# OliBomby/Mapperatorinator

Hardware: AMD Instinct MI355X
Metric: beatmap event-tokens/sec (mel + osuT5 encoder + greedy AR decode), whole job (higher is better)
Workload: dtype bf16; 1 GPU; osuT5-base bf16, batch=32 x 10 s chunks per GPU, 384 greedy tokens per chunk, mel+encoder+cross-KV+AR decode (BASELINE configs[1]); chunks_per_gpu=32, src_frames=1251, vocab=1849, parallelism=chunk-sharded x1, all_gather of token streams

## Files before the change

### mapperatorinator_amd/csrc/decode_kernels.hpp

```cpp
#pragma once
#include <type_traits>

#include "internal.hpp"

namespace mh {
namespace dec {

#ifdef MH_PHASE_STAMPS
__device__ unsigned long long g_stamps[16 * 16 * 2];
#define MH_STAMP0() unsigned long long mh_t0_ = 0; if (blockIdx.x == 0 && threadIdx.x == 0) mh_t0_ = clock64()
#define MH_STAMP(kid, i)                                                              \
  do {                                                                                \
    if (blockIdx.x == 0 && threadIdx.x == 0) {                                        \
      atomicAdd(&g_stamps[((kid) * 16 + (i)) * 2], (unsigned long long)clock64() - mh_t0_); \
      atomicAdd(&g_stamps[((kid) * 16 + (i)) * 2 + 1], 1ull);                         \
    }                                                                                 \
  } while (0)
#else
#define MH_STAMP0() do {} while (0)
#define MH_STAMP(kid, i) do {} while (0)
#endif
enum { KID_GEMV = 0 , KID_SELF = 10, KID_CROSS = 11, KID_SAMPLE = 12 };

typedef __attribute__((ext_vector_type(4))) unsigned int u32x4_t;
typedef __attribute__((ext_vector_type(2))) unsigned int u32x2_t;
template <typename T> __device__ inline void load8_stream(const T* p, float (&o)[8]);
template <> __device__ inline void load8_stream<bf16_t>(const bf16_t* p, float (&o)[8]) {
  const u32x4_t v = __builtin_nontemporal_load(reinterpret_cast<const u32x4_t*>(p));
#pragma unroll
  for (int i = 0; i < 4; ++i) {
    o[2 * i] = __uint_as_float(v[i] << 16);
    o[2 * i + 1] = __uint_as_float(v[i] & 0xffff0000u);
  }
}
template <> __device__ inline void load8_stream<float>(const float* p, float (&o)[8]) {
  const u32x4_t a = __builtin_nontemporal_load(reinterpret_cast<const u32x4_t*>(p));
  const u32x4_t b = __builtin_nontemporal_load(reinterpret_cast<const u32x4_t*>(p + 4));
#pragma unroll
  for (int i = 0; i < 4; ++i) { o[i] = __uint_as_float(a[i]); o[4 + i] = __uint_as_float(b[i]); }
}
struct fp8_t { uint8_t v; };
typedef __attribute__((ext_vector_type(2))) float f32x2_t;
template <> __device__ inline void load8_stream<fp8_t>(const fp8_t* p, float (&o)[8]) {
  const u32x2_t v = __builtin_nontemporal_load(reinterpret_cast<const u32x2_t*>(p));
#pragma unroll
  for (int i = 0; i < 2; ++i) {
    const f32x2_t lo = __builtin_amdgcn_cvt_pk_f32_fp8((int)v[i], false);
    const f32x2_t hi = __builtin_amdgcn_cvt_pk_f32_fp8((int)v[i], true);
    o[4 * i] = lo[0]; o[4 * i + 1] = lo[1]; o[4 * i + 2] = hi[0]; o[4 * i + 3] = hi[1];
  }
}
template <typename T> __device__ inline void store8(T* p, const float (&o)[8]);
template <> __device__ inline void store8<bf16_t>(bf16_t* p, const float (&o)[8]) {
  uint32_t w[4];
#pragma unroll
  for (int i = 0; i < 4; ++i) w[i] = pack_bf16x2(o[2 * i], o[2 * i + 1]);
  *reinterpret_cast<uint4*>(p) = make_uint4(w[0], w[1], w[2], w[3]);
}
template <> __device__ inline void store8<float>(float* p, const float (&o)[8]) {
  *reinterpret_cast<float4*>(p) = make_float4(o[0], o[1], o[2], o[3]);
  *reinterpret_cast<float4*>(p + 4) = make_float4(o[4], o[5], o[6], o[7]);
}

template <typename T> __device__ inline void store4(T* p, float a, float b, float c, float d);
template <> __device__ inline void store4<bf16_t>(bf16_t* p, float a, float b, float c, float d) {
  *reinterpret_cast<uint2*>(p) = make_uint2(pack_bf16x2(a, b), pack_bf16x2(c, d));
}
template <> __device__ inline void store4<float>(float* p, float a, float b, float c, float d) {
  *reinterpret_cast<float4*>(p) = make_float4(a, b, c, d);
}

#define MH_LOADS_ISSUED() do {} while (0)


template <typename U>
__device__ inline void store_wt(U* p, U v) { __hip_atomic_store(p, v, __ATOMIC_RELAXED, __HIP_MEMORY_SCOPE_AGENT); }
__device__ inline void store16_wt(void* p, u32x4_t v) { asm volatile("global_store_dwordx4 %0, %1, off sc1" : : "v"(p), "v"(v) : "memory"); }
__device__ inline void store8_wt(void* p, u32x2_t v) { asm volatile("global_store_dwordx2 %0, %1, off sc1" : : "v"(p), "v"(v) : "memory"); }
template <typename TO>
__device__ inline void store_piece_wt(TO* dst, const float* v, int n, int nvalid) {
  const bool whole = nvalid == n && (reinterpret_cast<uintptr_t>(dst) & (n * sizeof(TO) - 1)) == 0;
  if (whole && sizeof(TO) == 4 && n == 4) {
    store16_wt(dst, u32x4_t{__float_as_uint(v[0]), __float_as_uint(v[1]), __float_as_uint(v[2]), __float_as_uint(v[3])});
  } else if (whole && sizeof(TO) == 2 && n == 8) {
    store16_wt(dst, u32x4_t{pack_bf16x2(v[0], v[1]), pack_bf16x2(v[2], v[3]), pack_bf16x2(v[4], v[5]), pack_bf16x2(v[6], v[7])});
  } else if (whole && sizeof(TO) == 2 && n == 4) {
    store8_wt(dst, u32x2_t{pack_bf16x2(v[0], v[1]), pack_bf16x2(v[2], v[3])});
  } else {
    for (int i = 0; i < nvalid; ++i) store_wt(dst + i, Elem<TO>::from_f32(v[i]));
  }
}

template <typename T>
__device__ inline void store_head_row_wt(T* dst, float val, float* patch) {
  const int lane = threadIdx.x & 63;
  constexpr int N = 16 / (int)sizeof(T);
  patch[lane] = val;
  __builtin_amdgcn_fence(__ATOMIC_RELEASE, "wavefront");
  __builtin_amdgcn_wave_barrier();
  __builtin_amdgcn_fence(__ATOMIC_ACQUIRE, "wavefront");
  if (lane < 64 / N) {
    float v[8];
#pragma unroll
    for (int i = 0; i < 8; ++i) v[i] = i < N ? patch[lane * N + i] : 0.f;
    store_piece_wt<T>(dst + lane * N, v, N, N);
  }
}
template <typename T>
__device__ inline void store_head_row_from_lds_wt(T* dst, const float* src, int t) {
  constexpr int N = 16 / (int)sizeof(T);
  if (t >= 0 && t < 64 / N) {
    float v[8];
#pragma unroll
    for (int i = 0; i < 8; ++i) v[i] = i < N ? src[t * N + i] : 0.f;
    store_piece_wt<T>(dst + t * N, v, N, N);
  }
}

enum { PRO_PLAIN = 0, PRO_RMSNORM = 1, PRO_LAYERNORM = 2 };
enum { SK_GEGLU = 2, SK_RESID = 3, SK_LOGITS = 4, SK_GELU_ERF = 5 };

struct SkinnyP {
  const void* A; int lda;
  const float* ln_w; float eps;
  const void* W; int ldw;
  int B, N, K;
  int nv;
  void* out; int ldo;
  float* h; int ldh;
  void* kc; void* vc;
  int H, tgt_len, inner;
  const int* pos;
  const float* bias;
  const float* ln_b;
};

template <typename T> struct VecOps;
template <> struct VecOps<bf16_t> {
  struct Raw { float4 a, b; };
  __device__ static inline Raw load_raw(const float* p) {
    Raw r;
    r.a = *reinterpret_cast<const float4*>(p);
    r.b = *reinterpret_cast<const float4*>(p + 4);
    return r;
  }
  __device__ static inline float sumsq(const Raw& x) {
    return (x.a.x * x.a.x + x.a.y * x.a.y) + (x.a.z * x.a.z + x.a.w * x.a.w) + (x.b.x * x.b.x + x.b.y * x.b.y) +
           (x.b.z * x.b.z + x.b.w * x.b.w);
  }
  __device__ static inline float sum(const Raw& x) { return (x.a.x + x.a.y) + (x.a.z + x.a.w) + (x.b.x + x.b.y) + (x.b.z + x.b.w); }
  __device__ static inline Raw centred(const Raw& x, float mu) {
    Raw r;
    r.a = make_float4(x.a.x - mu, x.a.y - mu, x.a.z - mu, x.a.w - mu);
    r.b = make_float4(x.b.x - mu, x.b.y - mu, x.b.z - mu, x.b.w - mu);
    return r;
  }
  __device__ static inline uint4 ln_frag(const Raw& x, const Raw& g, const Raw& b, float rs) {
    const uint32_t o0 = pack_bf16x2(x.a.x * rs * g.a.x + b.a.x, x.a.y * rs * g.a.y + b.a.y);
    const uint32_t o1 = pack_bf16x2(x.a.z * rs * g.a.z + b.a.z, x.a.w * rs * g.a.w + b.a.w);
    const uint32_t o2 = pack_bf16x2(x.b.x * rs * g.b.x + b.b.x, x.b.y * rs * g.b.y + b.b.y);
    const uint32_t o3 = pack_bf16x2(x.b.z * rs * g.b.z + b.b.z, x.b.w * rs * g.b.w + b.b.w);
    return make_uint4(o0, o1, o2, o3);
  }
  __device__ static inline uint4 norm_frag(const Raw& x, const Raw& g, float rs) {
    const uint32_t o0 = pack_bf16x2(g.a.x * (x.a.x * rs), g.a.y * (x.a.y * rs));
    const uint32_t o1 = pack_bf16x2(g.a.z * (x.a.z * rs), g.a.w * (x.a.w * rs));
    const uint32_t o2 = pack_bf16x2(g.b.x * (x.b.x * rs), g.b.y * (x.b.y * rs));
    const uint32_t o3 = pack_bf16x2(g.b.z * (x.b.z * rs), g.b.w * (x.b.w * rs));
    return make_uint4(o0, o1, o2, o3);
  }
  __device__ static inline f32x4_t mma(const uint4& a, const uint4& b, f32x4_t c) {
    union U { uint4 u; bf16x8_t f; };
    U ua, ub;
    ua.u = a; ub.u = b;
    return __builtin_amdgcn_mfma_f32_16x16x32_bf16(ua.f, ub.f, c, 0, 0, 0);
  }
};
template <> struct VecOps<float> {
  struct Raw { float4 a; };
  __device__ static inline Raw load_raw(const float* p) {
    Raw r;
    r.a = *reinterpret_cast<const float4*>(p);
    return r;
  }
  __device__ static inline float sumsq(const Raw& x) { return (x.a.x * x.a.x + x.a.y * x.a.y) + (x.a.z * x.a.z + x.a.w * x.a.w); }
  __device__ static inline float sum(const Raw& x) { return (x.a.x + x.a.y) + (x.a.z + x.a.w); }
  __device__ static inline Raw centred(const Raw& x, float mu) {
    Raw r;
    r.a = make_float4(x.a.x - mu, x.a.y - mu, x.a.z - mu, x.a.w - mu);
    return r;
  }
  __device__ static inline uint4 ln_frag(const Raw& x, const Raw& g, const Raw& b, float rs) {
    return make_uint4(__float_as_uint(x.a.x * rs * g.a.x + b.a.x), __float_as_uint(x.a.y * rs * g.a.y + b.a.y),
                      __float_as_uint(x.a.z * rs * g.a.z + b.a.z), __float_as_uint(x.a.w * rs * g.a.w + b.a.w));
  }
  __device__ static inline uint4 norm_frag(const Raw& x, const Raw& g, float rs) {
    return make_uint4(__float_as_uint(g.a.x * (x.a.x * rs)), __float_as_uint(g.a.y * (x.a.y * rs)),
                      __float_as_uint(g.a.z * (x.a.z * rs)), __float_as_uint(g.a.w * (x.a.w * rs)));
  }
  __device__ static inline f32x4_t mma(const uint4& a, const uint4& b, f32x4_t c) {
    c = __builtin_amdgcn_mfma_f32_16x16x4f32(__uint_as_float(a.x), __uint_as_float(b.x), c, 0, 0, 0);
    c = __builtin_amdgcn_mfma_f32_16x16x4f32(__uint_as_float(a.y), __uint_as_float(b.y), c, 0, 0, 0);
    c = __builtin_amdgcn_mfma_f32_16x16x4f32(__uint_as_float(a.z), __uint_as_float(b.z), c, 0, 0, 0);
    c = __builtin_amdgcn_mfma_f32_16x16x4f32(__uint_as_float(a.w), __uint_as_float(b.w), c, 0, 0, 0);
    return c;
  }
};

constexpr int kGemvCH = 8;

#ifndef MH_GEMV_PROBE
#define MH_GEMV_PROBE 0
#endif

#define MH_GEMV_LEAD_PARAMS const void *A_, const void *W_, float *h_, const float *lnw_, int K_, int B_, int N_, int nv_
#define MH_GEMV_LEAD_ARGS(p) (p).A, (p).W, (p).h, (p).ln_w, (p).K, (p).B, (p).N, (p).nv
template <typename T, int MF, int NWV, int PRO, int EPI, bool BIAS = false>
__global__ __launch_bounds__(NWV * 64) __attribute__((amdgpu_waves_per_eu(NWV / 4, 4)))
void gemv_kernel(MH_GEMV_LEAD_PARAMS, SkinnyP p) {
  p.A = A_; p.W = W_; p.h = h_; p.ln_w = lnw_; p.K = K_; p.lda = K_; p.ldw = K_; p.B = B_; p.N = N_; p.nv = nv_;
  if (EPI == SK_RESID) p.ldh = N_;
  constexpr int VEC = Elem<T>::kVec;
  constexpr int KB = 4 * VEC;
  constexpr int CH = kGemvCH;
  typedef typename VecOps<T>::Raw Raw;
  constexpr bool LINES = (MF == 1 && PRO == PRO_PLAIN);
  constexpr int CP = CH / 2;
  constexpr int PATCH = 16 * 144;
  constexpr bool NORM = PRO != PRO_PLAIN, LN = PRO == PRO_LAYERNORM;
  constexpr bool RLINES = (MF == 1 && NORM && sizeof(T) == 2);
  __shared__ __attribute__((aligned(16))) unsigned char Lw[(LINES || RLINES) ? NWV * PATCH : 16];
  __shared__ f32x4_t red[NWV * MF * 64];
  __shared__ float ssw[NORM ? NWV : 1][MF * 16];
  __shared__ float ssw2[LN ? NWV : 1][MF * 16];
  __shared__ __attribute__((aligned(16))) float lnw[NORM ? 1024 : 4];
  __shared__ __attribute__((aligned(16))) float lnb[LN ? 1024 : 4];

  MH_STAMP0();
  constexpr int KID = KID_GEMV + EPI * 2 + (NWV == 8 ? 1 : 0);
  const int tid = threadIdx.x, lane = tid & 63, wid = tid >> 6;
  const int l15 = lane & 15, lg = lane >> 4;
  const int nv = p.nv;
  float4 lnraw = make_float4(0.f, 0.f, 0.f, 0.f), lnbraw = make_float4(0.f, 0.f, 0.f, 0.f);
  if (NORM) {
    const int i4 = tid * 4 < p.K ? tid * 4 : 0;
    lnraw = *reinterpret_cast<const float4*>(p.ln_w + i4);
    if (LN) lnbraw = *reinterpret_cast<const float4*>(p.ln_b + i4);
  }
  int wrow, ocol;
  bool wload;
  if (EPI == SK_GEGLU) {
    ocol = blockIdx.x * 8 + (l15 & 7);
    const int oc = ocol < p.N / 2 ? ocol : p.N / 2 - 1;
    wrow = (oc >> 4) * 32 + (l15 >> 3) * 16 + (oc & 15);
    wload = true;
  } else {
    ocol = blockIdx.x * nv + l15;
    wrow = ocol < p.N ? ocol : p.N - 1;
    wload = l15 < nv;
  }
  const T* Wp = reinterpret_cast<const T*>(p.W) + (long)wrow * p.ldw + lg * VEC;
  int arow[MF];
#pragma unroll
  for (int f = 0; f < MF; ++f) arow[f] = (f * 16 + l15) < p.B ? (f * 16 + l15) : p.B - 1;

  constexpr int UPW = (MF * 4 + NWV - 1) / NWV;
  const bool col_ok = (EPI == SK_GEGLU) ? (l15 < 8 && ocol < p.N / 2) : (l15 < nv && ocol < p.N);
  float oldh[UPW];
#pragma unroll
  for (int u = 0; u < UPW; ++u) oldh[u] = 0.f;
  constexpr int PROBE = MH_GEMV_PROBE;
  float bias_v = 0.f;
  if (BIAS) bias_v = p.bias[ocol < p.N ? ocol : p.N - 1];
#define MH_LOAD_OLDH()                                                                                                        \
  do {                                                                                                                        \
    _Pragma("unroll") for (int u = 0; u < UPW; ++u) {                                                                         \
      const int unit = wid + u * NWV;                                                                                         \
      const int row = (unit >> 2) * 16 + lg * 4 + (unit & 3);                                                                 \
      if (unit < MF * 4) oldh[u] = p.h[(long)(row < p.B ? row : p.B - 1) * p.ldh + (ocol < p.N ? ocol : p.N - 1)];          \
    }                                                                                                                         \
  } while (0)
  if (EPI == SK_RESID && l15 < nv && !(PROBE & 4)) MH_LOAD_OLDH();
  f32x4_t acc[MF];
#pragma unroll
  for (int f = 0; f < MF; ++f) acc[f] = f32x4_t{0.f, 0.f, 0.f, 0.f};
  const int nkb = p.K / KB;

  auto kblock = [](int kb0, int c) -> int { return PRO == PRO_PLAIN ? 2 * (kb0 + NWV * (c >> 1)) + (c & 1) : kb0 + NWV * c; };
  int kb0 = wid;
  if constexpr (LINES) {
    const int npair = nkb >> 1;
    unsigned char* patch = Lw + wid * PATCH;
    const int r8 = lane >> 3, c16 = (lane & 7) * 16;
    const unsigned char* Ab = reinterpret_cast<const unsigned char*>(p.A) + c16;
    const long rx = (long)(r8 < p.B ? r8 : p.B - 1) * p.lda * (long)sizeof(T);
    const long ry = (long)(8 + r8 < p.B ? 8 + r8 : p.B - 1) * p.lda * (long)sizeof(T);
    for (int pw0 = wid; pw0 < npair + wid; pw0 += NWV * CP) {
      uint4 wv[CH], xa[CP], ya[CP];
#pragma unroll
      for (int c = 0; c < CH; ++c) wv[c] = make_uint4(0, 0, 0, 0);
      if (wload && !(PROBE & 2)) {
#pragma unroll
        for (int c = 0; c < CH; ++c) {
          const int pw = pw0 + NWV * (c >> 1);
          wv[c] = *reinterpret_cast<const uint4*>(Wp + (2 * (pw < npair ? pw : npair - 1) + (c & 1)) * KB);
        }
      }
#pragma unroll
      for (int cp = 0; cp < CP; ++cp) {
        const int pw = pw0 + NWV * cp;
        const long off = (long)(pw < npair ? pw : npair - 1) * 128;
        xa[cp] = *reinterpret_cast<const uint4*>(Ab + rx + off);
        ya[cp] = *reinterpret_cast<const uint4*>(Ab + ry + off);
      }
      MH_LOADS_ISSUED();
      MH_LOADS_ISSUED();
    MH_STAMP(KID, 0);
#pragma unroll
      for (int cp = 0; cp < CP; ++cp) {
        const uint32_t keep = (pw0 + NWV * cp < npair) ? 0xffffffffu : 0u;
        *reinterpret_cast<uint4*>(patch + r8 * 144 + c16) = xa[cp];
        *reinterpret_cast<uint4*>(patch + (8 + r8) * 144 + c16) = ya[cp];
#pragma unroll
        for (int j = 0; j < 2; ++j) {
          uint4 a = *reinterpret_cast<const uint4*>(patch + l15 * 144 + (j * 4 + lg) * 16);
          a = make_uint4(a.x & keep, a.y & keep, a.z & keep, a.w & keep);
          acc[0] = VecOps<T>::mma(a, wv[cp * 2 + j], acc[0]);
        }
      }
    }
  } else
  do {
    uint4 wv[CH];
    uint4 av[PRO == PRO_PLAIN ? CH : 1][PRO == PRO_PLAIN ? MF : 1];
    Raw hraw[NORM ? CH : 1][NORM ? MF : 1];
#pragma unroll
    for (int c = 0; c < CH; ++c) wv[c] = make_uint4(0, 0, 0, 0);
    if (wload && !(PROBE & 2)) {
#pragma unroll
      for (int c = 0; c < CH; ++c) {
        const int kb = kblock(kb0, c);
        wv[c] = *reinterpret_cast<const uint4*>(Wp + (kb < nkb ? kb : nkb - 1) * KB);
      }
    }
#pragma unroll
    for (int c = 0; c < CH; ++c) {
      const int kb = kblock(kb0, c);
      const int kel = (kb < nkb ? kb : nkb - 1) * KB;
      if (PROBE & 1) {
#pragma unroll
        for (int f = 0; f < MF; ++f) {
          if (PRO == PRO_PLAIN) av[c][f] = make_uint4(kel, lane, c, f);
          else hraw[c][f] = VecOps<T>::load_raw(lnw + ((kel + lane) & 1020));
        }
      } else if (PRO == PRO_PLAIN && (PROBE & 128)) {
#pragma unroll
        for (int f = 0; f < MF; ++f)
          av[c][f] = *reinterpret_cast<const uint4*>(reinterpret_cast<const T*>(p.A) + ((long)((c * NWV + wid) % (p.K * 16 / (64 * VEC))) * 64 + lane) * VEC);
      } else if (PRO == PRO_PLAIN) {
#pragma unroll
        for (int f = 0; f < MF; ++f)
          av[c][f] = *reinterpret_cast<const uint4*>(reinterpret_cast<const T*>(p.A) + (long)arow[f] * p.lda + kel + lg * VEC);
      } else if (!RLINES) {
#pragma unroll
        for (int f = 0; f < MF; ++f)
          hraw[c][f] = VecOps<T>::load_raw(reinterpret_cast<const float*>(p.A) + (long)arow[f] * p.lda + kel + lg * VEC);
      }
    }
    uint4 xr[RLINES ? CH : 1], yr[RLINES ? CH : 1];
    if (RLINES) {
      const int r8 = lane >> 3;
      const unsigned char* Ab = reinterpret_cast<const unsigned char*>(p.A) + (lane & 7) * 16;
      const long rx = (long)(r8 < p.B ? r8 : p.B - 1) * p.lda * 4, ry = (long)(8 + r8 < p.B ? 8 + r8 : p.B - 1) * p.lda * 4;
#pragma unroll
      for (int c = 0; c < CH; ++c) {
        const int kb = kb0 + NWV * c;
        const long off = (long)(kb < nkb ? kb : nkb - 1) * 128;
        xr[c] = *reinterpret_cast<const uint4*>(Ab + rx + off);
        yr[c] = *reinterpret_cast<const uint4*>(Ab + ry + off);
      }
    }
    MH_LOADS_ISSUED();
    MH_STAMP(KID, 0);
    if (RLINES) {
      unsigned char* patch = Lw + wid * PATCH;
      const int r8 = lane >> 3, c16 = (lane & 7) * 16;
#pragma unroll
      for (int c = 0; c < CH; ++c) {
        *reinterpret_cast<uint4*>(patch + r8 * 144 + c16) = xr[c];
        *reinterpret_cast<uint4*>(patch + (8 + r8) * 144 + c16) = yr[c];
        hraw[c][0] = VecOps<T>::load_raw(reinterpret_cast<const float*>(patch + l15 * 144 + lg * 32));
      }
    }
    float rsr[MF];
    if (LN) {
#pragma unroll
      for (int f = 0; f < MF; ++f) {
        float q = 0.f;
#pragma unroll
        for (int c = 0; c < CH; ++c) q += (kb0 + NWV * c < nkb) ? VecOps<T>::sum(hraw[c][f]) : 0.f;
        q += __shfl_xor(q, 16, 64);
        q += __shfl_xor(q, 32, 64);
        if (lg == 0) ssw[wid][f * 16 + l15] = q;
      }
      if (tid * 4 < p.K) { *reinterpret_cast<float4*>(lnw + tid * 4) = lnraw; *reinterpret_cast<float4*>(lnb + tid * 4) = lnbraw; }
      __syncthreads();
#pragma unroll
      for (int f = 0; f < MF; ++f) {
        float su = 0.f;
#pragma unroll
        for (int w = 0; w < NWV; ++w) su += ssw[w][f * 16 + l15];
        const float mu = su / (float)p.K;
        float q = 0.f;
#pragma unroll
        for (int c = 0; c < CH; ++c) {
          hraw[c][f] = VecOps<T>::centred(hraw[c][f], mu);
          q += (kb0 + NWV * c < nkb) ? VecOps<T>::sumsq(hraw[c][f]) : 0.f;
        }
        q += __shfl_xor(q, 16, 64);
        q += __shfl_xor(q, 32, 64);
        if (lg == 0) ssw2[wid][f * 16 + l15] = q;
      }
      __syncthreads();
#pragma unroll
      for (int f = 0; f < MF; ++f) {
        float ss = 0.f;
#pragma unroll
        for (int w = 0; w < NWV; ++w) ss += ssw2[w][f * 16 + l15];
        rsr[f] = rsqrtf(ss / (float)p.K + p.eps);
      }
    } else if (PRO == PRO_RMSNORM) {
#pragma unroll
      for (int f = 0; f < MF; ++f) {
        float q = 0.f;
#pragma unroll
        for (int c = 0; c < CH; ++c) q += (kb0 + NWV * c < nkb) ? VecOps<T>::sumsq(hraw[c][f]) : 0.f;
        q += __shfl_xor(q, 16, 64);
        q += __shfl_xor(q, 32, 64);
        if (lg == 0) ssw[wid][f * 16 + l15] = q;
      }
      if (tid * 4 < p.K) *reinterpret_cast<float4*>(lnw + tid * 4) = lnraw;
      __syncthreads();
#pragma unroll
      for (int f = 0; f < MF; ++f) {
        float ss = 0.f;
#pragma unroll
        for (int w = 0; w < NWV; ++w) ss += ssw[w][f * 16 + l15];
        rsr[f] = rsqrtf(ss / (float)p.K + p.eps);
      }
    }
#pragma unroll
    for (int c = 0; c < CH; ++c) {
      const int kbc = kblock(kb0, c);
      const uint32_t keep = (kbc < nkb) ? 0xffffffffu : 0u;
      const int kc_el = ((kbc < nkb) ? kbc : nkb - 1) * KB + lg * VEC;
#pragma unroll
      for (int f = 0; f < MF; ++f) {
        uint4 a;
        if (PRO == PRO_PLAIN) a = av[c][f];
        else if (LN) a = VecOps<T>::ln_frag(hraw[c][f], VecOps<T>::load_raw(lnw + kc_el), VecOps<T>::load_raw(lnb + kc_el), rsr[f]);
        else a = VecOps<T>::norm_frag(hraw[c][f], VecOps<T>::load_raw(lnw + kc_el), rsr[f]);
        a = make_uint4(a.x & keep, a.y & keep, a.z & keep, a.w & keep);
        acc[f] = VecOps<T>::mma(a, wv[c], acc[f]);
      }
    }
    kb0 += NWV * (PRO == PRO_PLAIN ? CP : CH);
  } while (kblock(kb0, 0) < nkb);

  if (!(PROBE & 8)) {
#pragma unroll
    for (int f = 0; f < MF; ++f) red[(wid * MF + f) * 64 + lane] = acc[f];
  }
  MH_STAMP(KID, 1);
  if (!(PROBE & 8)) __syncthreads();
  MH_STAMP(KID, 2);

  const float* redf = reinterpret_cast<const float*>(red);
#pragma unroll
  for (int u = 0; u < UPW; ++u) {
    const int unit = wid + u * NWV;
    if (unit >= MF * 4) break;
    const int ef = unit >> 2, r = unit & 3;
    float v = 0.f;
    if (PROBE & 8) {
      v = acc[0][0] + acc[MF - 1][3];
    } else {
#pragma unroll
      for (int w = 0; w < NWV; ++w) v += redf[((w * MF + ef) * 64 + lane) * 4 + r];
    }
    const int row = ef * 16 + lg * 4 + r;
    const bool ok = col_ok && row < p.B && (!(PROBE & 16) || p.B < 0);
    if (BIAS) v += bias_v;
    if (EPI == SK_GELU_ERF) {
      if (ok) store_wt(reinterpret_cast<T*>(p.out) + (long)row * p.ldo + ocol, Elem<T>::from_f32(0.5f * v * (1.0f + erff(v * 0.70710678118654752f))));
    } else if (EPI == SK_GEGLU) {
      const float lin = __shfl_down(v, 8, 16);
      if (ok) store_wt(reinterpret_cast<T*>(p.out) + (long)row * p.ldo + ocol, Elem<T>::from_f32(gelu_tanh(v) * lin));
    } else if (EPI == SK_LOGITS) {
      if (ok) store_wt(reinterpret_cast<float*>(p.out) + (long)row * p.ldo + ocol, v);
    } else if (EPI == SK_RESID) {
      if (ok) store_wt(p.h + (long)row * p.ldh + ocol, oldh[u] + v);
    }
  }
  MH_STAMP(KID, 3);
#undef MH_LOAD_OLDH
}

struct Partial {
  float m, l;
  float acc[8];
};
__device__ inline void partial_init(Partial& s) {
  s.m = -1e30f; s.l = 0.f;
#pragma unroll
  for (int i = 0; i < 8; ++i) s.acc[i] = 0.f;
}
template <typename T>
__device__ inline void partial_merge_groups(Partial& s) {
  float mw = s.m;
#pragma unroll
  for (int o = 8; o < 64; o <<= 1) mw = fmaxf(mw, __shfl_xor(mw, o, 64));
  const float f = fexp<T>(s.m - mw);
  s.l *= f;
#pragma unroll
  for (int i = 0; i < 8; ++i) s.acc[i] *= f;
#pragma unroll
  for (int o = 8; o < 64; o <<= 1) {
    s.l += __shfl_xor(s.l, o, 64);
#pragma unroll
    for (int i = 0; i < 8; ++i) s.acc[i] += __shfl_xor(s.acc[i], o, 64);
  }
  s.m = mw;
}

template <typename T, int U, typename E = T>
__device__ inline void attend_keys(Partial& st, const float (&q)[8], const E* kbase, const E* vbase, int j0,
                                   int jend, int jstride, const float* bias_row, int pos, const uint8_t* mask_row,
                                   int P, float scale, int jmin = 0) {
  const int c8 = (threadIdx.x & 7) * 8;
  for (int j = j0; j < jend; j += jstride * U) {
    float s[U];
    float kv[U][8];
#pragma unroll
    for (int u = 0; u < U; ++u) {
      const int jj = j + u * jstride;
      const int jc = jj < jend ? jj : j;
      load8_stream<E>(kbase + (long)jc * 64 + c8, kv[u]);
    }
    float vv[U][8];
#pragma unroll
    for (int u = 0; u < U; ++u) {
      const int jj = j + u * jstride;
      const int jc = jj < jend ? jj : j;
      load8_stream<E>(vbase + (long)jc * 64 + c8, vv[u]);
    }
    float bv[U];
    int mv[U];
#pragma unroll
    for (int u = 0; u < U; ++u) { bv[u] = 0.f; mv[u] = 1; }
    if (bias_row) {
#pragma unroll
      for (int u = 0; u < U; ++u) {
        const int jj = j + u * jstride;
        bv[u] = bias_row[pos - (jj < jend ? jj : j)];
      }
    }
    if (mask_row) {
#pragma unroll
      for (int u = 0; u < U; ++u) {
        const int jj = j + u * jstride;
        const int jm = jj < P ? jj : P - 1;
        const int mval = mask_row[jm];
        mv[u] = (jj < P) ? mval : 1;
      }
    }
    float cmax = -INFINITY;
#pragma unroll
    for (int u = 0; u < U; ++u) {
      const int jj = j + u * jstride;
      float d = 0.f;
#pragma unroll
      for (int i = 0; i < 8; ++i) d += q[i] * kv[u][i];
      d = group_sum<8>(d) * scale + bv[u];
      const bool ok = (jj < jend) && (jj >= jmin) && (mv[u] != 0);
      d = ok ? d : -INFINITY;
      s[u] = d;
      cmax = fmaxf(cmax, d);
    }
    const float mn = fmaxf(st.m, cmax);
    const float fa = fexp<T>(st.m - mn);
    st.l *= fa;
#pragma unroll
    for (int i = 0; i < 8; ++i) st.acc[i] *= fa;
#pragma unroll
    for (int u = 0; u < U; ++u) {
      const float pu = fexp<T>(s[u] - mn);
      st.l += pu;
#pragma unroll
      for (int i = 0; i < 8; ++i) st.acc[i] += pu * vv[u][i];
    }
    st.m = mn;
  }
}

struct SelfAttnP {
  const void* q; int ldq;
  const void* kc; const void* vc;
  const float* bias;
  const uint8_t* prompt_mask; int P;
  void* out; int ldo;
  int B, H, tgt_len;
  const int* pos;
  const float* qkv_bias; const float* rope; float scale; int window;
};

template <typename T, int NW = 4>
__device__ inline void block_merge(const Partial& st, float (*sm)[66], float& m, float& l, float& a) {
  const int lane = threadIdx.x & 63, wid = threadIdx.x >> 6;
  const int c8 = (lane & 7) * 8, g = lane >> 3;
  if (g == 0) {
    if (lane == 0) { sm[wid][0] = st.m; sm[wid][1] = st.l; }
#pragma unroll
    for (int i = 0; i < 8; ++i) sm[wid][2 + c8 + i] = st.acc[i];
  }
  __syncthreads();
  m = -1e30f; l = 0.f; a = 0.f;
  if (threadIdx.x < 64) {
    const int d = threadIdx.x;
    m = sm[0][0];
#pragma unroll
    for (int w = 1; w < NW; ++w) m = fmaxf(m, sm[w][0]);
#pragma unroll
    for (int w = 0; w < NW; ++w) {
      const float f = fexp<T>(sm[w][0] - m);
      l += sm[w][1] * f;
      a += sm[w][2 + d] * f;
    }
  }
}

struct CrossAttnP {
  const void* q; int ldq;
  const void* k; const void* v;
  void* out; int ldo;
  int B, H, L;
  int kv_B;
  const float* kscale; const float* vscale;
  unsigned long long* tstamp; const int* pos; int ts_ring, ts_layers, ts_layer;
  const float* q_bias; float scale;
};

__device__ inline void cross_pair_of_block(const CrossAttnP& p, int blk, int& b, int& h) {
  if (p.kv_B > 0) {
    const int q2 = blk >> 1;
    b = (blk & 1) * p.kv_B + q2 / p.H;
    h = q2 % p.H;
  } else {
    b = blk / p.H;
    h = blk % p.H;
  }
}

struct HeadProjP {
  const float* h; int ldh;
  const float* ln_w; float eps;
  const void* W; int ldw;
  int d;
  const float* ln_b;
};

template <typename T> struct Raw8;
template <> struct Raw8<bf16_t> {
  uint4 v;
  __device__ inline void load(const bf16_t* p) { v = *reinterpret_cast<const uint4*>(p); }
  __device__ inline void unpack(float (&o)[8]) const {
    const uint32_t w[4] = {v.x, v.y, v.z, v.w};
#pragma unroll
    for (int i = 0; i < 4; ++i) { o[2 * i] = __uint_as_float(w[i] << 16); o[2 * i + 1] = __uint_as_float(w[i] & 0xffff0000u); }
  }
};
template <> struct Raw8<float> {
  float4 a, b;
  __device__ inline void load(const float* p) { a = *reinterpret_cast<const float4*>(p); b = *reinterpret_cast<const float4*>(p + 4); }
  __device__ inline void unpack(float (&o)[8]) const {
    o[0] = a.x; o[1] = a.y; o[2] = a.z; o[3] = a.w; o[4] = b.x; o[5] = b.y; o[6] = b.z; o[7] = b.w;
  }
};

template <typename T, bool LN = false>
struct NormRow {
  float x, g, bb;
  __device__ inline void issue_weight(const HeadProjP& hp) {
    const int tid = threadIdx.x;
    g = hp.ln_w[tid < hp.d ? tid : hp.d - 1];
    if (LN) bb = hp.ln_b[tid < hp.d ? tid : hp.d - 1];
  }
  __device__ inline void issue_row(const HeadProjP& hp, int b) {
    const int tid = threadIdx.x;
    x = hp.h[(long)b * hp.ldh + (tid < hp.d ? tid : hp.d - 1)];
  }
  __device__ inline void issue(const HeadProjP& hp, int b) { issue_row(hp, b); issue_weight(hp); }
  __device__ inline void finish(const HeadProjP& hp, float* xn, float* red16) {
    const int tid = threadIdx.x;
    if (LN) {
      const float su = wave_sum(tid < hp.d ? x : 0.f);
      if ((tid & 63) == 0) red16[tid >> 6] = su;
      __syncthreads();
      float tot = 0.f;
#pragma unroll
      for (int w = 0; w < 16; ++w) tot += red16[w];
      x -= tot / (float)hp.d;
      __syncthreads();
    }
    const float sq = wave_sum(tid < hp.d ? x * x : 0.f);
    if ((tid & 63) == 0) red16[tid >> 6] = sq;
    __syncthreads();
    float tot = 0.f;
#pragma unroll
    for (int w = 0; w < 16; ++w) tot += red16[w];
    const float rs = rsqrtf(tot / (float)hp.d + hp.eps);
    if (tid < hp.d) xn[tid] = Elem<T>::to_f32(Elem<T>::from_f32(LN ? x * rs * g + bb : g * (x * rs)));
    __syncthreads();
  }
};

template <typename T, int KC, int NP>
struct HeadProj {
  Raw8<T> raw[NP][KC];
  __device__ inline void load(const HeadProjP& hp, const int (&row0)[NP]) {
    const int tid = threadIdx.x, o = tid >> 4, ks = tid & 15;
#pragma unroll
    for (int q = 0; q < NP; ++q) {
      const T* wp = reinterpret_cast<const T*>(hp.W) + (long)(row0[q] + o) * hp.ldw + ks * 8;
#pragma unroll
      for (int c = 0; c < KC; ++c) raw[q][c].load(wp + c * 128);
    }
    MH_LOADS_ISSUED();
  }
  __device__ inline void load3(const HeadProjP& hp, const int (&row0)[3]) {
    const int tid = threadIdx.x, o = tid >> 4, ks = tid & 15;
#pragma unroll
    for (int q = 0; q < (NP < 3 ? NP : 3); ++q) {
      const T* wp = reinterpret_cast<const T*>(hp.W) + (long)(row0[q] + o) * hp.ldw + ks * 8;
#pragma unroll
      for (int c = 0; c < KC; ++c) raw[q][c].load(wp + c * 128);
    }
  }
  __device__ inline void apply(const float* xn, float (*out)[64], const float* bias = nullptr, const int* row0 = nullptr) const {
    const int tid = threadIdx.x, o = tid >> 4, ks = tid & 15;
#pragma unroll
    for (int q = 0; q < NP; ++q) {
      float acc = 0.f;
#pragma unroll
      for (int c = 0; c < KC; ++c) {
        float w[8];
        raw[q][c].unpack(w);
        const float4 x0 = *reinterpret_cast<const float4*>(xn + c * 128 + ks * 8);
        const float4 x1 = *reinterpret_cast<const float4*>(xn + c * 128 + ks * 8 + 4);
        acc += x0.x * w[0] + x0.y * w[1] + x0.z * w[2] + x0.w * w[3] + x1.x * w[4] + x1.y * w[5] + x1.z * w[6] + x1.w * w[7];
      }
      acc = group_sum<16>(acc);
      if (bias) acc += bias[row0[q] + o];
      if (ks == 0) out[q][o] = Elem<T>::to_f32(Elem<T>::from_f32(acc));
    }
  }
};

template <typename T, int KC, int U, bool F8 = false, bool WH = false, bool LN = false>
__global__ __launch_bounds__(1024) __attribute__((amdgpu_waves_per_eu(8, 8)))
void dec_cross_attn_q_kernel(const float* h_, const float* lnw_, const void* W_, const void* k_, const void* v_, int H_, int L_, int d_,
                             int kvB_, CrossAttnP p, HeadProjP hp) {
  hp.h = h_; hp.ln_w = lnw_; hp.W = W_; hp.ldh = d_; hp.ldw = d_; hp.d = d_;
  p.k = k_; p.v = v_; p.H = H_; p.L = L_; p.kv_B = kvB_;
  constexpr int NW = 16;
  __shared__ float sm[NW][66];
  __shared__ __attribute__((aligned(16))) float xn[1024];
  __shared__ float qs[1][64];
  __shared__ float red16[16];
  const int lane = threadIdx.x & 63, wid = threadIdx.x >> 6;
  int b, h;
  cross_pair_of_block(p, blockIdx.x, b, h);
  MH_STAMP0();
  const int c8 = (lane & 7) * 8, g = lane >> 3;
  const int row0[1] = {h * 64};
  const int kvb = p.kv_B > 0 ? b % p.kv_B : (p.kv_B < 0 ? b / -p.kv_B : b);
  typedef typename std::conditional<F8, fp8_t, T>::type E;
  const E* kb = reinterpret_cast<const E*>(p.k) + ((long)kvb * p.H + h) * p.L * 64;
  const E* vb = reinterpret_cast<const E*>(p.v) + ((long)kvb * p.H + h) * p.L * 64;
  HeadProj<T, KC, 1> proj;
  NormRow<T, LN> nrow;
  nrow.issue(hp, b);
  if (sizeof(T) == 2) proj.load(hp, row0);
  unsigned long long t_start = 0;
  if (p.tstamp && threadIdx.x == 0) t_start = (unsigned long long)wall_clock64();
  nrow.finish(hp, xn, red16);
  MH_STAMP(KID_CROSS, 0);
  if (sizeof(T) != 2) proj.load(hp, row0);
  proj.apply(xn, qs, WH ? p.q_bias : nullptr, row0);
  __syncthreads();
  MH_STAMP(KID_CROSS, 1);
  float q[8];
#pragma unroll
  for (int i = 0; i < 8; ++i) q[i] = qs[0][c8 + i];
  const float ks = (F8 ? p.kscale[kvb * p.H + h] : 1.0f) * (WH ? p.scale : 1.0f), vs = F8 ? p.vscale[kvb * p.H + h] : 1.0f;
  Partial st;
  partial_init(st);
  attend_keys<T, U, E>(st, q, kb, vb, wid * 8 + g, p.L, 8 * NW, nullptr, 0, nullptr, 0, ks);
  MH_STAMP(KID_CROSS, 2);
  partial_merge_groups<T>(st);
  float m, l, a;
  block_merge<T, NW>(st, sm, m, l, a);
  MH_STAMP(KID_CROSS, 3);
  if (threadIdx.x < 64)
    store_head_row_wt<T>(reinterpret_cast<T*>(p.out) + (long)b * p.ldo + h * 64, l > 0.f ? a / l * vs : 0.f, &sm[0][0]);
  if (p.tstamp && threadIdx.x == 0 && *p.pos < p.ts_ring) {
    unsigned long long* slot = p.tstamp + 2 * ((long)(*p.pos) * p.ts_layers + p.ts_layer);
    atomicMin(slot, t_start);
    atomicMax(slot + 1, (unsigned long long)wall_clock64());
  }
}

template <typename T, int KC, bool WH = false, bool LN = false>
__global__ __launch_bounds__(1024) __attribute__((amdgpu_waves_per_eu(4, 4)))
void dec_self_attn_qkv_kernel(const float* h_, const float* lnw_, const void* W_, const int* pos_,
                                                                 const void* kc_, const void* vc_, int H_, int d_, SelfAttnP p,
                                                                 HeadProjP hp) {
  hp.h = h_; hp.ln_w = lnw_; hp.W = W_; hp.ldh = d_; hp.ldw = d_; hp.d = d_;
  p.pos = pos_; p.kc = kc_; p.vc = vc_; p.H = H_;
  const int inner = H_ * 64;
  constexpr int NW = 16;
  __shared__ float sm[NW][66];
  __shared__ __attribute__((aligned(16))) float xn[1024];
  __shared__ float qkv[3][64];
  __shared__ float red16[16];
  MH_STAMP0();
  const int lane = threadIdx.x & 63, wid = threadIdx.x >> 6;
  const int b = blockIdx.x / p.H, h = blockIdx.x % p.H;
  const int c8 = (lane & 7) * 8, g = lane >> 3;
  NormRow<T, LN> nrow;
  nrow.issue(hp, b);
  const int pos = *p.pos;
  constexpr bool kAllAtOnce = sizeof(T) == 2 && KC <= 7;
  HeadProj<T, KC, kAllAtOnce ? 3 : 1> proj;
  const int row03[3] = {h * 64, inner + h * 64, 2 * inner + h * 64};
  const float* bias_row = WH ? nullptr : p.bias + (long)h * p.tgt_len;
  const uint8_t* mask_row = p.prompt_mask ? p.prompt_mask + (long)b * p.P : nullptr;
  const float bias0 = WH ? 0.f : bias_row[0];
  float rope_c = 1.f, rope_s = 0.f;
  if (WH) {
    rope_c = p.rope[(long)pos * 64 + (threadIdx.x & 31)];
    rope_s = p.rope[(long)pos * 64 + 32 + (threadIdx.x & 31)];
  }
  const int new_key_mask = (mask_row && pos < p.P) ? (int)mask_row[pos < p.P ? pos : 0] : 1;
  nrow.finish(hp, xn, red16);
  const float* qb = WH ? p.qkv_bias : nullptr;
  if (kAllAtOnce) {
    proj.load3(hp, row03);
    proj.apply(xn, qkv, qb, row03);
  } else {
#pragma unroll
    for (int q3 = 0; q3 < 3; ++q3) {
      const int row0[1] = {q3 * inner + h * 64};
      HeadProj<T, KC, 1> proj1;
      proj1.load(hp, row0);
      proj1.apply(xn, qkv + q3, qb, row0);
    }
  }
  __syncthreads();
  if (WH) {
    float rot = 0.f;
    const int t = threadIdx.x;
    if (t < 128) {
      const float* x = qkv[t >> 6];
      const int i = t & 31;
      const float x1 = x[i], x2 = x[i + 32];
      rot = (t & 32) ? x2 * rope_c + x1 * rope_s : x1 * rope_c - x2 * rope_s;
    }
    __syncthreads();
    if (t < 128) qkv[t >> 6][t & 63] = Elem<T>::to_f32(Elem<T>::from_f32(rot));
    __syncthreads();
  }
  MH_STAMP(KID_SELF, 0);
  T* kcache = reinterpret_cast<T*>(const_cast<void*>(p.kc)) + ((long)b * p.H + h) * p.tgt_len * 64;
  T* vcache = reinterpret_cast<T*>(const_cast<void*>(p.vc)) + ((long)b * p.H + h) * p.tgt_len * 64;
  store_head_row_from_lds_wt<T>(kcache + (long)pos * 64, qkv[1], (int)threadIdx.x - 64);
  store_head_row_from_lds_wt<T>(vcache + (long)pos * 64, qkv[2], (int)threadIdx.x - 128);
  float q[8];
#pragma unroll
  for (int i = 0; i < 8; ++i) q[i] = qkv[0][c8 + i];
  Partial st;
  partial_init(st);
  const float sc = WH ? p.scale : 1.0f;
  int j_first = 0;
  if (WH && p.window > 0 && pos - p.window > 0) j_first = (pos - p.window) & ~(8 * NW - 1);
  attend_keys<T, 2>(st, q, kcache, vcache, j_first + wid * 8 + g, pos, 8 * NW, bias_row, pos, mask_row, p.P, sc,
                    (WH && p.window > 0) ? pos - p.window : 0);
  MH_STAMP(KID_SELF, 1);
  partial_merge_groups<T>(st);
  float m, l, a;
  block_merge<T, NW>(st, sm, m, l, a);
  MH_STAMP(KID_SELF, 2);
  if (threadIdx.x < 64) {
    const int d = threadIdx.x;
    float sn = wave_sum(qkv[0][d] * qkv[1][d]) * sc + bias0;
    if (new_key_mask == 0) sn = -INFINITY;
    const float mn = fmaxf(m, sn);
    const float fa = fexp<T>(m - mn), fb = fexp<T>(sn - mn);
    l = l * fa + fb;
    a = a * fa + qkv[2][d] * fb;
    store_head_row_wt<T>(reinterpret_cast<T*>(p.out) + (long)b * p.ldo + h * 64, l > 0.f ? a / l : 0.f, &sm[0][0]);
  }
}

}
}
```

Before: 45120 event-tokens/s.

## Prefetch self-attention KV cache during QKV projection and double-buffer key loads

The fused decode self-attention kernel now issues its first batch of K/V cache, bias and mask loads before the QKV head projection runs, so their latency overlaps the projection math. The attention loop is replaced by one that holds keys in registers and prefetches the next group while computing the current one. This costs more registers, which may hurt occupancy or cause spills under the fixed 1024-thread, 8-waves bound. Out-of-range keys are clamped to the last valid row and zeroed by masking.

```diff
diff --git a/mapperatorinator_amd/csrc/decode_kernels.hpp b/mapperatorinator_amd/csrc/decode_kernels.hpp
--- a/mapperatorinator_amd/csrc/decode_kernels.hpp
+++ b/mapperatorinator_amd/csrc/decode_kernels.hpp
@@ -603,6 +603,105 @@
   }
 }
 
+template <typename T, int U>
+struct CachedKeys {
+  static constexpr int NV = 8 * (int)sizeof(T) / 16;
+  u32x4_t k[U][NV], v[U][NV];
+  float bias[U];
+  int mask[U];
+  __device__ inline void request(const T* kbase, const T* vbase, const float* bias_row, const uint8_t* mask_row, int P,
+                                 int j, int jstride, int pos) {
+    const int c8 = (threadIdx.x & 7) * 8;
+    const int last = pos > 0 ? pos - 1 : 0;
+#pragma unroll
+    for (int u = 0; u < U; ++u) {
+      const int jj = j + u * jstride;
+      const long off = (long)(jj < last ? jj : last) * 64 + c8;
+#pragma unroll
+      for (int i = 0; i < NV; ++i) k[u][i] = __builtin_nontemporal_load(reinterpret_cast<const u32x4_t*>(kbase + off) + i);
+    }
+#pragma unroll
+    for (int u = 0; u < U; ++u) {
+      const int jj = j + u * jstride;
+      const long off = (long)(jj < last ? jj : last) * 64 + c8;
+#pragma unroll
+      for (int i = 0; i < NV; ++i) v[u][i] = __builtin_nontemporal_load(reinterpret_cast<const u32x4_t*>(vbase + off) + i);
+    }
+#pragma unroll
+    for (int u = 0; u < U; ++u) { bias[u] = 0.f; mask[u] = 1; }
+    if (bias_row) {
+#pragma unroll
+      for (int u = 0; u < U; ++u) {
+        const int jj = j + u * jstride;
+        bias[u] = bias_row[pos - (jj < last ? jj : last)];
+      }
+    }
+    if (mask_row) {
+#pragma unroll
+      for (int u = 0; u < U; ++u) {
+        const int jj = j + u * jstride;
+        mask[u] = mask_row[jj < P ? jj : P - 1];
+      }
+    }
+  }
+  __device__ static inline void unpack(const u32x4_t (&r)[NV], uint32_t keep, float (&o)[8]) {
+    if (sizeof(T) == 2) {
+#pragma unroll
+      for (int i = 0; i < 4; ++i) {
+        const uint32_t w = r[0][i] & keep;
+        o[2 * i] = __uint_as_float(w << 16);
+        o[2 * i + 1] = __uint_as_float(w & 0xffff0000u);
+      }
+    } else {
+#pragma unroll
+      for (int i = 0; i < 4; ++i) { o[i] = __uint_as_float(r[0][i] & keep); o[4 + i] = __uint_as_float(r[NV - 1][i] & keep); }
+    }
+  }
+};
+
+template <typename T, int U>
+__device__ inline void attend_cached_keys(Partial& st, const float (&q)[8], CachedKeys<T, U> cur, const T* kbase, const T* vbase,
+                                          int j0, int pos, int jstride, const float* bias_row, const uint8_t* mask_row, int P,
+                                          float scale, int jmin) {
+  for (int j = j0; j < pos; j += jstride * U) {
+    CachedKeys<T, U> nxt = cur;
+    if (j + jstride * U < pos) nxt.request(kbase, vbase, bias_row, mask_row, P, j + jstride * U, jstride, pos);
+    float s[U];
+    bool ok[U];
+    float cmax = -INFINITY;
+#pragma unroll
+    for (int u = 0; u < U; ++u) {
+      const int jj = j + u * jstride;
+      float kv[8];
+      CachedKeys<T, U>::unpack(cur.k[u], 0xffffffffu, kv);
+      float d = 0.f;
+#pragma unroll
+      for (int i = 0; i < 8; ++i) d += q[i] * kv[i];
+      d = group_sum<8>(d) * scale + cur.bias[u];
+      ok[u] = (jj < pos) && (jj >= jmin) && (cur.mask[u] != 0 || jj >= P);
+      d = ok[u] ? d : -INFINITY;
+      s[u] = d;
+      cmax = fmaxf(cmax, d);
+    }
+    const float mn = fmaxf(st.m, cmax);
+    const float fa = fexp<T>(st.m - mn);
+    st.l *= fa;
+#pragma unroll
+    for (int i = 0; i < 8; ++i) st.acc[i] *= fa;
+#pragma unroll
+    for (int u = 0; u < U; ++u) {
+      const float pu = fexp<T>(s[u] - mn);
+      float vv[8];
+      CachedKeys<T, U>::unpack(cur.v[u], ok[u] ? 0xffffffffu : 0u, vv);
+      st.l += pu;
+#pragma unroll
+      for (int i = 0; i < 8; ++i) st.acc[i] += pu * vv[i];
+    }
+    st.m = mn;
+    cur = nxt;
+  }
+}
+
 struct SelfAttnP {
   const void* q; int ldq;
   const void* kc; const void* vc;
@@ -746,17 +845,20 @@
       for (int c = 0; c < KC; ++c) raw[q][c].load(wp + c * 128);
     }
   }
+  template <bool REREAD = false>
   __device__ inline void apply(const float* xn, float (*out)[64], const float* bias = nullptr, const int* row0 = nullptr) const {
     const int tid = threadIdx.x, o = tid >> 4, ks = tid & 15;
 #pragma unroll
     for (int q = 0; q < NP; ++q) {
+      const float* xq = xn + ks * 8;
+      if (REREAD) asm volatile("" : "+v"(xq));
       float acc = 0.f;
 #pragma unroll
       for (int c = 0; c < KC; ++c) {
         float w[8];
         raw[q][c].unpack(w);
-        const float4 x0 = *reinterpret_cast<const float4*>(xn + c * 128 + ks * 8);
-        const float4 x1 = *reinterpret_cast<const float4*>(xn + c * 128 + ks * 8 + 4);
+        const float4 x0 = *reinterpret_cast<const float4*>(xq + c * 128);
+        const float4 x1 = *reinterpret_cast<const float4*>(xq + c * 128 + 4);
         acc += x0.x * w[0] + x0.y * w[1] + x0.z * w[2] + x0.w * w[3] + x1.x * w[4] + x1.y * w[5] + x1.z * w[6] + x1.w * w[7];
       }
       acc = group_sum<16>(acc);
@@ -853,16 +955,26 @@
   }
   const int new_key_mask = (mask_row && pos < p.P) ? (int)mask_row[pos < p.P ? pos : 0] : 1;
   nrow.finish(hp, xn, red16);
+  MH_STAMP(KID_SELF, 0);
+  T* kcache = reinterpret_cast<T*>(const_cast<void*>(p.kc)) + ((long)b * p.H + h) * p.tgt_len * 64;
+  T* vcache = reinterpret_cast<T*>(const_cast<void*>(p.vc)) + ((long)b * p.H + h) * p.tgt_len * 64;
+  int j_first = 0;
+  if (WH && p.window > 0 && pos - p.window > 0) j_first = (pos - p.window) & ~(8 * NW - 1);
+  const int j0 = j_first + wid * 8 + g;
+  CachedKeys<T, 2> keys;
+  constexpr bool kEarlyKeys = sizeof(T) == 2 ? (kAllAtOnce && KC <= (WH ? 5 : 6)) : KC <= 4;
   const float* qb = WH ? p.qkv_bias : nullptr;
   if (kAllAtOnce) {
     proj.load3(hp, row03);
-    proj.apply(xn, qkv, qb, row03);
+    if (kEarlyKeys && j0 < pos) keys.request(kcache, vcache, bias_row, mask_row, p.P, j0, 8 * NW, pos);
+    proj.template apply<kEarlyKeys>(xn, qkv, qb, row03);
   } else {
 #pragma unroll
     for (int q3 = 0; q3 < 3; ++q3) {
       const int row0[1] = {q3 * inner + h * 64};
       HeadProj<T, KC, 1> proj1;
       proj1.load(hp, row0);
+      if (kEarlyKeys && q3 == 0 && j0 < pos) keys.request(kcache, vcache, bias_row, mask_row, p.P, j0, 8 * NW, pos);
       proj1.apply(xn, qkv + q3, qb, row0);
     }
   }
@@ -880,9 +992,7 @@
     if (t < 128) qkv[t >> 6][t & 63] = Elem<T>::to_f32(Elem<T>::from_f32(rot));
     __syncthreads();
   }
-  MH_STAMP(KID_SELF, 0);
-  T* kcache = reinterpret_cast<T*>(const_cast<void*>(p.kc)) + ((long)b * p.H + h) * p.tgt_len * 64;
-  T* vcache = reinterpret_cast<T*>(const_cast<void*>(p.vc)) + ((long)b * p.H + h) * p.tgt_len * 64;
+  MH_STAMP(KID_SELF, 1);
   store_head_row_from_lds_wt<T>(kcache + (long)pos * 64, qkv[1], (int)threadIdx.x - 64);
   store_head_row_from_lds_wt<T>(vcache + (long)pos * 64, qkv[2], (int)threadIdx.x - 128);
   float q[8];
@@ -891,15 +1001,14 @@
   Partial st;
   partial_init(st);
   const float sc = WH ? p.scale : 1.0f;
-  int j_first = 0;
-  if (WH && p.window > 0 && pos - p.window > 0) j_first = (pos - p.window) & ~(8 * NW - 1);
-  attend_keys<T, 2>(st, q, kcache, vcache, j_first + wid * 8 + g, pos, 8 * NW, bias_row, pos, mask_row, p.P, sc,
-                    (WH && p.window > 0) ? pos - p.window : 0);
-  MH_STAMP(KID_SELF, 1);
+  if (!kEarlyKeys && j0 < pos) keys.request(kcache, vcache, bias_row, mask_row, p.P, j0, 8 * NW, pos);
+  attend_cached_keys<T, 2>(st, q, keys, kcache, vcache, j0, pos, 8 * NW, bias_row, mask_row, p.P, sc,
+                           (WH && p.window > 0) ? pos - p.window : 0);
+  MH_STAMP(KID_SELF, 2);
   partial_merge_groups<T>(st);
   float m, l, a;
   block_merge<T, NW>(st, sm, m, l, a);
-  MH_STAMP(KID_SELF, 2);
+  MH_STAMP(KID_SELF, 3);
   if (threadIdx.x < 64) {
     const int d = threadIdx.x;
     float sn = wave_sum(qkv[0][d] * qkv[1][d]) * sc + bias0;
```

After: 41960 event-tokens/s. -7.0%, worse.
